# moddyz/stereo-to-multiview-cuda

Measured on AMD Instinct MI355X. Metric: stereo->8-view frames/sec @1080p d=64; cost-agg HBM GB/s vs roofline, higher is better.
Workload: dtype f32; 1 GPU; 1920x1080 synthetic stereo frame, D=64, zd=32, full stereo->8-view frame: cost init + cross aggregation + WTA + DCC/IRV x5/bilateral + 6 DIBR views + interlacing, one frame per GPU per step; stages=3, usd=34, lsd=17, views=8, aggregation=matrix pipe (stm_kernels_aggm.hip)

## Files before the change

include/stm_hip.h:

```cpp
#ifndef STM_HIP_H
#define STM_HIP_H

#ifdef __cplusplus
extern "C" {
#endif
#if defined(STM_BUILD) && defined(__GNUC__)
#pragma GCC visibility push(default)
#endif

int         stm_version(void);
void        stm_set_stream(void *hip_stream);
void       *stm_get_stream(void);
void        stm_set_error_mode(int mode);
const char *stm_last_error(void);
void        stm_release_workspace(void);
void        stm_prof_enable(int on);
void        stm_prof_reset(void);
int         stm_prof_read(const char *kernel, float *total_ms);
void        stm_set_agg_variant(int v);
int         stm_agg_path(int num_disp, int zero_disp, int num_rows, int num_cols, int usd, int stages);
void        stm_set_irv_paper_ratio(int on);
int         stm_set_irv_chunk(int entries);
int         stm_irv_path(int num_rows, int num_cols, int usd, int iterations, int device_flavour, int with_dcc);
int         stm_set_lens(int mode, double pitch, double slope, double centre);
int         stm_set_depth(int mode, float gain, float conv);
int         stm_set_depth_auto(float disp_lo, float disp_hi, float max_gain, int clip_permille, float rate, float *d_state);
int         stm_set_layout(int layout, int tiles_x, int tiles_y, int order, int filter);
void        stm_get_layout(int *out);
int         stm_set_output(int format, int matrix, int pitch, int uv_row);
void        stm_get_output(int out[4]);
void        stm_set_quilt_lds_limit(int bytes);
int         stm_set_packing(int packing, int swap, int filter, int gap);
void        stm_get_packing(int *out);
void        stm_set_ref_quirks(int on);

void stm_ci_adcensus(unsigned char *img_l, unsigned char *img_r, float **cost_l, float **cost_r,
                     float ad_coeff, float census_coeff, int num_disp, int zero_disp,
                     int num_rows, int num_cols, int elem_sz);
void stm_d_ci_adcensus(unsigned char *d_img_l, unsigned char *d_img_r,
                       float **d_adcensus_cost_l, float **d_adcensus_cost_r,
                       float **h_adcensus_cost_l, float **h_adcensus_cost_r,
                       float *d_adcensus_cost_memory,
                       float ad_coeff, float census_coeff, int num_disp, int zero_disp,
                       int num_rows, int num_cols, int elem_sz);

void stm_ca_cross(unsigned char *img, unsigned char **cross, float **cost, float **acost,
                  float ucd, float lcd, int usd, int lsd,
                  int num_disp, int num_rows, int num_cols, int elem_sz);
void stm_d_ca_cross(unsigned char *d_img, float **d_cost,
                    float **d_acost, float **h_acost, float *d_acost_memory,
                    unsigned char **d_cross,
                    float ucd, float lcd, int usd, int lsd,
                    int num_disp, int num_rows, int num_cols, int elem_sz);
// ... 227 lines not shown
```

stereo-to-multiview-cuda_amd/_lib.py:

```python
import ctypes as C
import os

HERE = os.path.dirname(os.path.abspath(__file__))
LIB_PATH = os.path.join(HERE, "libstm_hip.so")
if os.environ.get("STM_LIB") == "timing":
    LIB_PATH = os.path.join(HERE, "libstm_hip_timing.so")

u8p = C.POINTER(C.c_uint8)
f32p = C.POINTER(C.c_float)
u32p = C.POINTER(C.c_uint32)
u8pp = C.POINTER(u8p)
f32pp = C.POINTER(f32p)
vp = C.c_void_p
i, f, d = C.c_int, C.c_float, C.c_double

PROTOS = {
    "stm_version": ([], i),
    "stm_set_stream": ([vp], None),
    "stm_get_stream": ([], vp),
    "stm_set_error_mode": ([i], None),
    "stm_last_error": ([], C.c_char_p),
    "stm_release_workspace": ([], None),
    "stm_prof_enable": ([i], None),
    "stm_prof_reset": ([], None),
    "stm_prof_read": ([C.c_char_p, f32p], i),
    "stm_set_agg_variant": ([i], None),
    "stm_agg_path": ([i, i, i, i, i, i], i),
    "stm_set_irv_paper_ratio": ([i], None),
    "stm_set_irv_chunk": ([i], i),
    "stm_irv_path": ([i, i, i, i, i, i], i),
    "stm_set_ref_quirks": ([i], None),
    "stm_set_lens": ([i, d, d, d], i),
    "stm_set_layout": ([i, i, i, i, i], i),
    "stm_get_layout": ([C.POINTER(C.c_int)], None),
    "stm_set_output": ([i, i, i, i], i),
    "stm_get_output": ([C.POINTER(C.c_int)], None),
    "stm_set_quilt_lds_limit": ([i], None),
    "stm_set_packing": ([i, i, i, i], i),
    "stm_get_packing": ([C.POINTER(C.c_int)], None),
    "stm_set_depth": ([i, f, f], i),
    "stm_set_depth_auto": ([f, f, f, i, f, vp], i),
    "stm_ci_adcensus": ([u8p, u8p, f32pp, f32pp, f, f, i, i, i, i, i], None),
    "stm_d_ci_adcensus": ([vp, vp, vp, vp, f32pp, f32pp, vp, f, f, i, i, i, i, i], None),
    "stm_ca_cross": ([u8p, u8pp, f32pp, f32pp, f, f, i, i, i, i, i, i], None),
    "stm_d_ca_cross": ([vp, vp, vp, f32pp, vp, vp, f, f, i, i, i, i, i, i], None),
    "stm_dc_wta": ([f32pp, f32p, i, i, i, i], None),
    "stm_d_dc_wta": ([vp, vp, i, i, i, i], None),
    "stm_dc_subpixel": ([f32pp, f32p, i, i, i, i], None),
    "stm_d_dc_subpixel": ([vp, vp, i, i, i, i], None),
    "stm_dc_hslo": ([f32pp, f32p, u8p, u8p, f, f, f, i, i, i, i, i], None),
    "stm_d_dc_hslo": ([vp, vp, vp, vp, f, f, f, i, i, i, i, i], None),
    "stm_dr_dcc": ([u8p, u8p, f32p, f32p, i, i], None),
    "stm_d_dr_dcc": ([vp, vp, vp, vp, i, i], None),
    "stm_dr_irv": ([f32p, u8p, u8pp, i, f, i, i, i, i, i, i], None),
    "stm_d_dr_irv": ([vp, vp, vp, i, f, i, i, i, i, i, i], None),
    "stm_dr_interp": ([f32p, u8p, u8p, i, i, i], None),
    "stm_d_dr_interp": ([vp, vp, vp, i, i, i], None),
    "stm_filter_bilateral_1": ([f32p, i, f, f, i, i, i], None),
    "stm_d_filter_bilateral_1": ([vp, i, f, f, i, i, i], None),
    "stm_filter_gaussian_1": ([f32p, i, f, i, i], None),
# ... 95 lines not shown
```

stereo-to-multiview-cuda_amd/csrc/stm_api.hip:

```cpp
#include "stm_common.h"
#include <initializer_list>
#include <mutex>
#include "../../include/stm_hip.h"

#include <map>
#include <stdio.h>
#include <stdlib.h>
#include <string.h>
#include <tuple>
#include <vector>

using namespace stm;

namespace {

struct DevTable {
    float *d = nullptr;
    size_t n = 0;
};
std::map<std::tuple<int, int, float, float>, DevTable> g_tables;

int cur_dev()
{
    int dev = 0;
// ... 96 lines not shown
        }
    return true;
}


void core_ci(const u8 *d_img_l, const u8 *d_img_r, Vol cl, Vol cr, uint32_t *pk_l, uint32_t *pk_r, float ad_coeff,
             float census_coeff, int D, int zd, int H, int W, int elem_sz, bool packed_ready = false,
             uint32_t **census_out = nullptr, uint32_t *const *census_ready = nullptr)
{
    size_t HW = (size_t)H * W;
    uint32_t *cen_l = census_ready ? census_ready[0] : Workspace::get<uint32_t>(HW), *cen_r = census_ready ? census_ready[1] : Workspace::get<uint32_t>(HW);
    if (!packed_ready) {
        launch_pack_bgrx(d_img_l, pk_l, H, W, elem_sz);
        launch_pack_bgrx(d_img_r, pk_r, H, W, elem_sz);
    }
    if (!census_ready) launch_census32_pair(pk_l, cen_l, pk_r, cen_r, H, W);
    if (census_out) {
        census_out[0] = cen_l;
        census_out[1] = cen_r;
        return;
    }
    const float *lut = rho_table(ad_coeff, census_coeff);
    launch_cost_init(pk_l, pk_r, cen_l, cen_r, cl, cr, lut, lut + 768, D, zd, H, W);
    if (ref_quirks()) launch_cost_quirks(pk_l, pk_r, cen_l, cen_r, cl, cr, lut, lut + 768, D, zd, H, W);
}

static bool agg_on_matrix_pipe(int usd, int H, int W) { return (agg_variant() / 10000) % 10 != 1 && aggm_supports(usd, H, W); }
static bool stages_hslo(int stages) { return (stages & 0x100) != 0; }
static bool stages_subpix(int stages) { return (stages & 0x200) != 0; }
int frame_agg_path(int D, int zd, int H, int W, int usd, int stages)
{
    if (D < 1 || H < 1 || W < 1 || !agg_on_matrix_pipe(usd, H, W)) return 0;
    return 1 | aggm_frame_path(D, zd, H, W, usd, stages_hslo(stages), stages_subpix(stages));
}
void core_agg(Vol cost, Vol scratch, const Arms &a, int D, int H, int W, int usd)
{
    if (agg_on_matrix_pipe(usd, H, W) && launch_aggm_stage(cost, cost, a.up, a.down, a.left, a.right, D, H, W, usd)) return;
    if (!scratch.base && !scratch.tab) scratch = vol_slab(Workspace::get<float>((size_t)D * H * W), (size_t)H * W);
    launch_agg_h(cost, scratch, a.left, a.right, D, H, W);
    launch_agg_v(scratch, cost, a.up, a.down, D, H, W, usd);
    launch_agg_v(cost, scratch, a.up, a.down, D, H, W, usd);
    launch_agg_h(scratch, cost, a.left, a.right, D, H, W);
}
Arms carve_arms(size_t HW)
{
    u8 *m = Workspace::get<u8>(4 * HW);
    return Arms{m, m + HW, m + 2 * HW, m + 3 * HW};
}
Arms arms_from_table(unsigned char **d_cross)
{
    u8 *h[4];
    STM_CHECK(hipMemcpyAsync(h, d_cross, sizeof h, hipMemcpyDeviceToHost, stream()));
    sync();
    return Arms{h[0], h[1], h[2], h[3]};
}

void core_bilateral(float *d_img, int radius, float sigma_color, float sigma_spatial, int H, int W, int D)
{
    size_t HW = (size_t)H * W;
    float *tmp = Workspace::get<float>(HW);
    launch_bilateral(d_img, tmp, gauss2d_table(radius, sigma_spatial), gauss1d_table(D, sigma_color), radius, H, W, D);
    STM_CHECK(hipMemcpyAsync(d_img, tmp, HW * sizeof(float), hipMemcpyDeviceToDevice, stream()));
}

void core_dbm(u8 *d_out, const u8 *d_l, const u8 *d_r, const float *disp_l, const float *disp_r, const float *mask_l,
              const float *mask_r, float shift, int H, int W, int elem_sz, int g_radius, float g_sigma, bool linear = false)
// ... 1345 lines not shown
}

bool frame_dims_ok(const char *fn, int num_rows, int num_cols_sbs, int num_cols, int num_rows_out, int num_cols_out, int elem_sz,
                   int num_views, int num_disp)
{
    return args_ok(fn, {{"num_rows", num_rows, 1}, {"num_cols_sbs", num_cols_sbs, 1}, {"num_cols", num_cols, 1},
                        {"num_rows_out", num_rows_out, 1}, {"num_cols_out", num_cols_out, 1}, {"elem_sz", elem_sz, 3},
                        {"num_views", num_views, 2}, {"num_disp", num_disp, 1}});
}

bool frame_packing_ok(const char *fn, int num_rows, int num_cols_sbs, int num_cols)
{
    const Packing pk = packing();
    return !pk.on() || packing_args_ok(fn, pk, num_rows, num_cols_sbs, num_cols, "num_cols", false, 0, 0, 0);
}
bool packing_unsupported(const char *fn)
{
    if (!packing().on()) return false;
    char msg[200];
    snprintf(msg, sizeof msg, "%s: a packing is set on this thread (stm_set_packing), which this call does not support: use d_adcensus_stm, "
             "d_adcensus_stm_t or d_adcensus_stm_nv12", fn);
    fail(msg, "packing", __FILE__, __LINE__);
    return true;
}

}

extern "C" {

int stm_agg_path(int num_disp, int zero_disp, int num_rows, int num_cols, int usd, int stages)
{
    return frame_agg_path(num_disp, zero_disp, num_rows, num_cols, usd, stages);
}

void stm_d_adcensus_stm(unsigned char *d_img_sbs, float *d_disp_l, float *d_disp_r, unsigned char *d_interlaced,
                        int num_rows, int num_cols_sbs, int num_cols, int num_rows_out, int num_cols_out, int elem_sz,
                        int num_views, float angle, int num_disp, int zero_disp, float ad_coeff, float census_coeff,
                        float ucd, float lcd, int usd, int lsd, int thresh_s, float thresh_h, int stages)
{
    if (!frame_dims_ok("d_adcensus_stm", num_rows, num_cols_sbs, num_cols, num_rows_out, num_cols_out, elem_sz, num_views, num_disp)) return;
    if (!frame_packing_ok("d_adcensus_stm", num_rows, num_cols_sbs, num_cols)) return;
    if (stages & 0x2000) {
        fail("d_adcensus_stm: stages 0x2000 (temporal stabilisation) needs the history arguments of d_adcensus_stm_t", "stages", __FILE__,
             __LINE__);
        return;
    }
    frame_device("d_adcensus_stm", d_img_sbs, d_disp_l, d_disp_r, d_interlaced, num_rows, num_cols_sbs, num_cols, num_rows_out, num_cols_out,
                 elem_sz, num_views, angle, num_disp, zero_disp, ad_coeff, census_coeff, ucd, lcd, usd, lsd, thresh_s, thresh_h, stages, nullptr);
}

void stm_d_adcensus_stm_t(unsigned char *d_img_sbs, float *d_disp_l, float *d_disp_r, unsigned char *d_interlaced,
                          int num_rows, int num_cols_sbs, int num_cols, int num_rows_out, int num_cols_out, int elem_sz,
                          int num_views, float angle, int num_disp, int zero_disp, float ad_coeff, float census_coeff,
                          float ucd, float lcd, int usd, int lsd, int thresh_s, float thresh_h, int stages,
                          unsigned char *d_prev_img_sbs, float *d_prev_disp_l, float *d_prev_disp_r, float alpha, int thresh_color,
                          float thresh_disp)
{
    const char *fn = "d_adcensus_stm_t";
    if (!frame_dims_ok(fn, num_rows, num_cols_sbs, num_cols, num_rows_out, num_cols_out, elem_sz, num_views, num_disp)) return;
    if (!frame_packing_ok(fn, num_rows, num_cols_sbs, num_cols)) return;
    TemporalHist hist = {d_prev_img_sbs, d_prev_disp_l, d_prev_disp_r, alpha, thresh_color, thresh_disp};
    bool run = false;
    if (stages & 0x2000) {
        const int nset = (d_prev_img_sbs != nullptr) + (d_prev_disp_l != nullptr) + (d_prev_disp_r != nullptr);
        const size_t HW = (size_t)num_rows * num_cols;
        if (!temporal_params_ok(fn, alpha, thresh_color, thresh_disp)) return;
// ... 503 lines not shown
```

stereo-to-multiview-cuda_amd/csrc/stm_common.h:

```cpp
#pragma once
#include <hip/hip_runtime.h>
#include <stddef.h>
#include <stdint.h>

typedef unsigned char u8;

namespace stm {

void fail(const char *what, const char *expr, const char *file, int line);
bool failed();
void clear_failed();
struct ApiNest { ApiNest(); ~ApiNest(); };
bool api_outermost();
void release_host_frame_bufs();
bool nv12_args_ok(const char *fn, int num_rows, int num_cols_sbs, int num_cols, const char *cols_name, int pitch_y, int pitch_uv, int matrix);
#define STM_CHECK(expr)                                                                  \
    do {                                                                                 \
        hipError_t _e = (expr);                                                          \
        if (_e != hipSuccess) ::stm::fail(hipGetErrorString(_e), #expr, __FILE__, __LINE__); \
    } while (0)
#define STM_CHECK_LAUNCH() STM_CHECK(hipGetLastError())
#define STM_LAUNCH(...)                                     \
    do {                                                    \
        if (!::stm::failed()) hipLaunchKernelGGL(__VA_ARGS__); \
// ... 222 lines not shown
                      const float *blend, u8 *out, int N, float y_interval, float inv_y_interval, int ymod, int Hin, int Win, int Hout,
                      int Wout, int elem_sz, int variant, bool linear = false);
void launch_mux(const u8 *const *d_views, u8 *out, int N, float y_interval, float inv_y_interval, int ymod,
                int Hin, int Win, int Hout, int Wout, int elem_sz, int variant);
void launch_mux_lens(const u8 *const *d_views, u8 *out, int N, const Lens &ln, int Hin, int Win, int Hout, int Wout, int elem_sz);
void launch_synth_mux_lens(const u8 *img_l, const u8 *img_r, const float *disp_l, const float *disp_r, const float *mask_l,
                           const float *mask_r, const float *blend, u8 *out, int N, const Lens &ln, int Hin, int Win, int Hout, int Wout,
                           int elem_sz, bool linear);
void launch_synth_mux_depth(const u8 *img_l, const u8 *img_r, const float *disp_l, const float *disp_r, const float *mask_l,
                            const float *mask_r, const float *blend, u8 *out, int N, const Lens &ln, float inv_y_interval, int ymod,
                            float gain, float conv, const float *state, int Hin, int Win, int Hout, int Wout, int elem_sz, bool linear);
void launch_quilt(const u8 *const *d_views, u8 *out, int N, const Layout &lo, int Hin, int Win, int Hout, int Wout, int elem_sz);
void launch_synth_quilt(const u8 *img_l, const u8 *img_r, const float *disp_l, const float *disp_r, const float *mask_l, const float *mask_r,
                        const float *blend, u8 *out, int N, const Layout &lo, int depth_mode, float gain, float conv, const float *state,
                        int Hin, int Win, int Hout, int Wout, int elem_sz, bool linear, const Nv12Out *nv = nullptr);
void launch_depth_fit(float *state, uint32_t *hist, const float *disp_l, const float *disp_r, int H, int W, float disp_lo, float disp_hi,
                      float max_gain, int clip_permille, float rate, bool fresh);
struct PQViews {
    const uint32_t *pk[2], *cen[2];
    float *a[2], *b[2];
    const u8 *armU[2], *armD[2], *armL[2], *armR[2];
    float *disp[2];
};
size_t pq_volume_floats(int D, int H, int W);
bool aggm_supports(int usd, int H, int W);
void launch_aggm_frame(const uint32_t *const *pk, const uint32_t *const *cen, const float *lut, float *const *vol_a, float *const *vol_b,
                       const u8 *const *armU, const u8 *const *armD, const u8 *const *armL, const u8 *const *armR, float *const *disp,
                       int D, int zd, int H, int W, int usd, bool keep_volume = false, uint32_t *htab_ready = nullptr, uint32_t *vtab_ready = nullptr,
                       bool v2_read_later = false);
size_t aggm_frame_htab_dwords(int D, int H, int W, int usd, bool keep_volume);
size_t aggm_frame_vtab_dwords(int D, int zd, int H, int W, int usd, bool keep_volume, bool v2_read_later, int *rec, int *top, bool *col);
bool aggm_frame_px(int D, int zd, int H, int W, int usd, bool keep_volume, bool v2_read_later);
int aggm_frame_path(int D, int zd, int H, int W, int usd, bool keep_volume, bool v2_read_later);
bool launch_aggm_stage(Vol in, Vol out, const u8 *armU, const u8 *armD, const u8 *armL, const u8 *armR, int D, int H, int W, int usd);
size_t aggm_stage_bytes(int D, int H, int W, int usd);
bool aggh_supports(int usd, int D);
size_t aggh_table_dwords(int nviews, int H, int W);
void launch_hwin_table(PQViews &v, int nviews, uint32_t *tab, int H, int W);
void launch_pq_hsr(PQViews &v, int nviews, const uint32_t *tab, int D, int zd, int H, int W, bool px = false);
bool aggv_supports(int usd);
int aggv_table_top();
int aggv_table_rec();
void launch_pq_v12q(PQViews &v, int nviews, const uint32_t *tab, int rec, int H, int W, int G, int NC);
void launch_pq_v12r(PQViews &v, int nviews, const uint32_t *tab, int H, int W, int G);
void launch_vcol_table(PQViews &v, int nviews, uint32_t *tab, int H, int W);
size_t aggv_col_table_dwords(int nviews, int H, int W);
void launch_to_pq(Vol in, float *pq, int D, int H, int W, uint32_t *odd = nullptr);
void launch_from_pq(const float *pq, Vol out, int D, int H, int W);
void launch_hslo_wta(int nviews, const Vol *cost, const u8 *const *img_a, const u8 *const *img_b, const int *osign,
                     float *const *disp, float T, float H1, float H2, int D, int zd, int H, int W, int elem_sz);
void launch_hslo_wta_pq(int nviews, float *const *cost_pq, float *const *acc_pq, const u8 *const *img_a, const u8 *const *img_b,
                        const int *osign, float *const *disp, float T, float H1, float H2, int D, int zd, int H, int W, int elem_sz);

void rho_luts(float ad_coeff, float census_coeff, float *lut_ad , float *lut_census );
void gaussian_kernel_2d(float *kernel, int radius, float sigma);
void gaussian_kernel_1d(float *kernel, int size, float sigma);
float mux_y_interval(int num_views, float angle, int elem_sz);

}
```

stereo-to-multiview-cuda_amd/csrc/stm_kernels_aggm.hip:

```cpp
#include "stm_hwin.h"

namespace stm {

typedef float f4 __attribute__((ext_vector_type(4)));

#define STM_MFMA16(m, b, acc, abid) __builtin_amdgcn_mfma_f32_16x16x1f32(m, b, acc, 2, abid, 0)
typedef float f16v __attribute__((ext_vector_type(16)));
typedef uint32_t u4v __attribute__((ext_vector_type(4)));
#define STM_MASKF(m) (__builtin_amdgcn_inverse_ballot_w64(m) ? 1.0f : 0.0f)
#define STM_BLOAD(rsrc, voff) __builtin_bit_cast(f4, __builtin_amdgcn_raw_buffer_load_b128(rsrc, voff, 0, 2))


template <int N> __device__ __forceinline__ float row_ror_f(float v)
{
    return __builtin_bit_cast(float, __builtin_amdgcn_update_dpp(0, __builtin_bit_cast(int, v), 0x120 + N, 0xf, 0xf, false));
}
template <int N> __device__ __forceinline__ int row_ror_i(int v) { return __builtin_amdgcn_update_dpp(0, v, 0x120 + N, 0xf, 0xf, false); }
__device__ __forceinline__ int wave_min_i(int v)
{
    v = min(v, row_ror_i<8>(v)); v = min(v, row_ror_i<4>(v)); v = min(v, row_ror_i<2>(v)); v = min(v, row_ror_i<1>(v));
    return min(min(__builtin_amdgcn_readlane(v, 0), __builtin_amdgcn_readlane(v, 16)),
               min(__builtin_amdgcn_readlane(v, 32), __builtin_amdgcn_readlane(v, 48)));
}
__device__ __forceinline__ int wave_max_i(int v)
// ... 636 lines not shown
#pragma unroll
                for (int cl = 0; cl < 4; ++cl) {
                    const f4 o = {acc[4 * cl], acc[4 * cl + 1], acc[4 * cl + 2], acc[4 * cl + 3]};
                    if (!STM_DBG(dbg, 4)) STM_BSTORE(rout[cl], (X0 >> 2) * 256 + l * 16, o);
                }
            } else {
#pragma unroll
                for (int k = 0; k < 16; ++k)
                    if (!STM_DBG(dbg, 4))
                        __builtin_amdgcn_raw_buffer_store_b32(__builtin_bit_cast(uint32_t, (float)acc[k]), rpx,
                                                              (X0 + 4 * lb + (k & 3)) * 256 + (16 * (k >> 2) + dd) * 4, 0, 2);
            }
        }
        if (more) STM_HC_COSTS((sq + 1) & 1, 4 * NW * (sq + 1) + NG - 4 * NW)
        __syncthreads();
        if (more) {
            int sl = slot0 + w;
            if (sl >= NJ) sl -= NJ;
#pragma unroll
            for (int k = 0; k < 4; ++k) tile[(k * NJ + sl) * 64 + l] = cst[k];
            STM_HC_STAGE(sq & 1)
            STM_HC_SN(sq + 1)
            slot0 += NW;
            if (slot0 >= NJ) slot0 -= NJ;
        }
        __syncthreads();
    }
  }
#undef STM_HC_FETCH
#undef STM_HC_STAGE
#undef STM_HC_COSTS
#undef STM_HC_ARMS
#undef STM_HC_SN
}

constexpr int VT_EV = 2 * 255 + 32;
__global__ __launch_bounds__(256) void stm_k_vwin_table(PQViews v, uint32_t *__restrict__ tab, int rec, int H, int W, int G, int nT, int top)
{
    __shared__ unsigned long long ev_all[4][VT_EV];
    const int l = threadIdx.x & 63, wv = threadIdx.x >> 6, g = blockIdx.x * 4 + wv, u = blockIdx.y, view = blockIdx.z;
    if (g >= G) return;
    unsigned long long *ev = ev_all[wv];
    const u8 *__restrict__ armU = view ? v.armU[1] : v.armU[0], *__restrict__ armD = view ? v.armD[1] : v.armD[0];
    const int b = l >> 4, i = l & 15, y = u * 16 + i, x = 4 * g + b;
    int s0 = 0, nn = 0;
    if (y < H && x < W) {
        const int aU = armU[(size_t)y * W + x], aD = armD[(size_t)y * W + x];
        s0 = y - aU;
        nn = aU + aD;
    }
    vwin_build(tab + ((size_t)(view * nT + u) * G + g) * rec, ev, u, top, s0, nn);
}

typedef __attribute__((address_space(4))) const uint32_t ctab32;
typedef __attribute__((address_space(4))) const unsigned long long ctab64;
struct V12Quad { f4 c; unsigned long long m0, m1, m2, m3; };
struct V12Sweep {
    const f4 *p;
    ctab64 *mk;
    int qs, n_it;
    V12Quad A;
};
#define STM_V12_LOAD(S, Q, RQ)                                                      \
    {                                                                               \
        Q.c = *S.p;                                                                 \
        Q.m0 = S.mk[0]; Q.m1 = S.mk[1]; Q.m2 = S.mk[2]; Q.m3 = S.mk[3];             \
// ... 229 lines not shown
static int hc_waves(int D, int zd, int usd)
{
    constexpr int NW = 8, NWC = 12;
    const int NC = (D + 15) / 16;
    const int HG = ((usd + 3) / 4 + 2) & ~1, NG = 4 * NW + 2 * HG, NGc = 4 * NWC + 2 * HG;
    int pad = zd > D - 1 - zd ? zd : D - 1 - zd;
    pad = (pad < 0 ? 0 : pad) + 15;
    const size_t smem_hc = (size_t)4 * NGc * 256 + 16 * NWC * 4 + 8 * NWC + (size_t)(2 * 16 * NWC + 2 * (16 * NWC + 2 * pad)) * 8 + (768 + 72) * 4;
    const size_t smem_hc8 = (size_t)4 * NG * 256 + 16 * NW * 4 + 8 * NW + (size_t)(2 * 16 * NW + 2 * (16 * NW + 2 * pad)) * 8 + (768 + 72) * 4;
    const bool hc_ok = (agg_variant() / 1000000) % 10 != 1 && (agg_variant() / 1000) % 10 == 0 && (NC <= 4 || (agg_variant() / 10) % 10 != 2);
    if (hc_ok && smem_hc <= 80 * 1024 && 16 * NWC + 2 * pad <= 64 * NWC) return NWC;
    if (hc_ok && smem_hc8 <= 80 * 1024 && 16 * NW + 2 * pad <= 64 * NW) return NW;
    return 0;
}

static int row_split(int nseg) { return nseg > 24 ? cdiv(nseg, 16) : 1; }
static bool chain_vregs(int usd) { return aggv_supports(usd) && (agg_variant() / 10000000) % 10 != 1; }
static bool chain_hregs(bool wta, int usd, int D) { return wta && aggh_supports(usd, D) && (agg_variant() / 100000000) % 10 != 1; }

static bool chain_px(bool from_costs, bool wta, int D, int zd, int usd)
{
    if (usd > 255) usd = 255;
    const int NC = (D + 15) / 16;
    return from_costs && NC == 4 && chain_vregs(usd) && (agg_variant() / 10000000) % 10 == 0 && chain_hregs(wta, usd, D) &&
           hc_waves(D, zd, usd) != 0;
}
bool aggm_frame_px(int D, int zd, int H, int W, int usd, bool keep_volume, bool v2_read_later)
{
    (void)H;
    (void)W;
    return !v2_read_later && chain_px(true, !keep_volume, D, zd, usd);
}

struct ChainPlan {
    bool regs, hregs;
    int hcw;
    int hc_nseg, hc_spl;
};
static ChainPlan chain_plan(bool from_costs, bool wta, int D, int zd, int W, int usd)
{
    ChainPlan c;
    c.regs = chain_vregs(usd);
    c.hregs = chain_hregs(wta, usd, D);
    const bool fuse_cost = from_costs && (agg_variant() / 1000000) % 10 != 1;
    c.hcw = fuse_cost ? hc_waves(D, zd, usd) : 0;
    c.hc_nseg = c.hcw ? cdiv(W, 16 * c.hcw) : 0;
    c.hc_spl = row_split(c.hc_nseg);
    return c;
}
int aggm_frame_path(int D, int zd, int H, int W, int usd, bool keep_volume, bool v2_read_later)
{
    if (usd > 255) usd = 255;
    const ChainPlan c = chain_plan(true, !keep_volume, D, zd, W, usd);
    return (aggm_frame_px(D, zd, H, W, usd, keep_volume, v2_read_later) ? 2 : 0) | (c.regs ? 4 : 0) | (c.hregs ? 8 : 0) | (c.hcw << 8) |
           (c.hc_spl > 1 ? 1 << 16 : 0);
}

static void aggm_chain(PQViews &v, int nviews, bool from_costs, bool wta, const float *lut, int D, int zd, int H, int W, int usd,
                       uint32_t *htab_ready = nullptr, uint32_t *vtab_ready = nullptr, bool px = false)
{
    const int G = (W + 3) / 4, NC = (D + 15) / 16;
    if (usd > 255) usd = 255;
    constexpr int NW = 8;
    const int HG = ((usd + 3) / 4 + 2) & ~1, NG = 4 * NW + 2 * HG;
    const int nseg = cdiv(W, 16 * NW), nblk = ((nseg * H * nviews + 7) / 8) * 8;
    const size_t smem_h = (size_t)4 * NG * 256 + 16 * NW * 4;
    const int dbgh = timing_knobs();
    int pad = zd > D - 1 - zd ? zd : D - 1 - zd;
    pad = (pad < 0 ? 0 : pad) + 15;
    const size_t smem_cost = smem_h + (size_t)(4 * NG * 4 + 4 * pad + 768 + 72) * 4;
    const bool fuse_cost = from_costs && (agg_variant() / 1000000) % 10 != 1;
    const int spl = row_split(nseg);
    const ChainPlan plan = chain_plan(from_costs, wta, D, zd, W, usd);
    const bool streaming = NG / 4 >= NW && (agg_variant() / 10) % 10 != 1 && (NC <= 4 || (agg_variant() / 10) % 10 != 2);
    constexpr int NTP = 3, TS = 16 * NTP;
    const int UQ = (usd + 3) & ~3, nT = (H + 15) / 16;
    const bool regs = plan.regs;
    const int rec = regs ? aggv_table_rec() : 8 + 8 * ((2 * usd + 21) / 4 + 2);
    const int LAG = (UQ + TS - 1) / TS + 1;
    const int RQ1 = (TS + 2 * UQ) / 4, RQ2 = (TS * (LAG + 1) + UQ) / 4;
    uint32_t *vtab = regs && vtab_ready ? vtab_ready : Workspace::get<uint32_t>(px ? aggv_col_table_dwords(nviews, H, W) : (size_t)nviews * nT * G * rec);
    const bool hregs = plan.hregs;
    uint32_t *htab = !hregs ? nullptr : htab_ready ? htab_ready : Workspace::get<uint32_t>(aggh_table_dwords(nviews, H, W));
    {
        if (!(regs && vtab_ready)) {
            ProfScope p("pq_vtab");
            if (px) launch_vcol_table(v, nviews, vtab, H, W);
            else STM_LAUNCH(stm_k_vwin_table, dim3(cdiv(G, 4), nT, nviews), dim3(256), 0, stream(), v, vtab, rec, H, W, G, nT, regs ? aggv_table_top() : -1);
            STM_CHECK_LAUNCH();
        }
        if (hregs && !htab_ready) {
            ProfScope p("pq_htab");
            launch_hwin_table(v, nviews, htab, H, W);
        }
    }
    if (from_costs && !fuse_cost) {
        ProfScope p("pq_cost");
        const size_t smem = (size_t)(2 * PC_TX + 2 * (PC_TX + 2 * pad) + 768 + 72) * 4;
        allow_lds_m((const void *)stm_k_pq_cost, smem);
        STM_LAUNCH(stm_k_pq_cost, dim3(cdiv(W, PC_TX), H, nviews), dim3(PC_TX), smem, stream(), v, lut, D, zd, H, W, G, NC, pad);
        STM_CHECK_LAUNCH();
    }
    {
        ProfScope p("pq_h");
        constexpr int NWC = 12;
        const int NGc = 4 * NWC + 2 * HG;
        const size_t smem_c12 = (size_t)4 * NGc * 256 + 16 * NWC * 4 + (size_t)(4 * NGc * 4 + 4 * pad + 768 + 72) * 4;
        const size_t smem_hc = (size_t)4 * NGc * 256 + 16 * NWC * 4 + 8 * NWC + (size_t)(2 * 16 * NWC + 2 * (16 * NWC + 2 * pad)) * 8 + (768 + 72) * 4;
        const int nsegc = cdiv(W, 16 * NWC);
        const size_t smem_hc8 = (size_t)4 * NG * 256 + 16 * NW * 4 + 8 * NW + (size_t)(2 * 16 * NW + 2 * (16 * NW + 2 * pad)) * 8 + (768 + 72) * 4;
        const int hcw = plan.hcw;
#define STM_HC_LAUNCH(NWX, PXS, GRID, SMEM, NSEG, SPL)                                                                                      \
    {                                                                                                                                     \
        allow_lds_m((const void *)stm_k_pq_hc<NWX, PXS>, SMEM);                                                                            \
        STM_LAUNCH((stm_k_pq_hc<NWX, PXS>), GRID, dim3(64 * NWX), SMEM, stream(), v, D, zd, H, W, G, NC, HG, NSEG, SPL, lut, pad, dbgh);    \
    }
        if (hcw == NWC) {
            const dim3 grid(nviews * H * plan.hc_spl);
            if (px) STM_HC_LAUNCH(NWC, true, grid, smem_hc, plan.hc_nseg, plan.hc_spl)
            else STM_HC_LAUNCH(NWC, false, grid, smem_hc, plan.hc_nseg, plan.hc_spl)
        } else if (hcw == NW) {
            const dim3 grid(nviews * H * plan.hc_spl);
            if (px) STM_HC_LAUNCH(NW, true, grid, smem_hc8, plan.hc_nseg, plan.hc_spl)
            else STM_HC_LAUNCH(NW, false, grid, smem_hc8, plan.hc_nseg, plan.hc_spl)
        } else if (fuse_cost && smem_c12 <= 80 * 1024 && (agg_variant() / 1000) % 10 != 1) {
            const int nblkc = ((nsegc * H * nviews + 7) / 8) * 8;
            allow_lds_m((const void *)stm_k_pq_h<NWC, false, true>, smem_c12);
            STM_LAUNCH((stm_k_pq_h<NWC, false, true>), dim3(nblkc), dim3(64 * NWC), smem_c12, stream(), v, D, zd, H, W, G, NC, HG, nsegc, dbgh, lut, pad, nviews);
        } else if (fuse_cost) {
            allow_lds_m((const void *)stm_k_pq_h<NW, false, true>, smem_cost);
            STM_LAUNCH((stm_k_pq_h<NW, false, true>), dim3(nblk), dim3(64 * NW), smem_cost, stream(), v, D, zd, H, W, G, NC, HG, nseg, dbgh, lut, pad, nviews);
        } else if (streaming) {
            allow_lds_m((const void *)stm_k_pq_hs<NW, false>, smem_h);
            STM_LAUNCH((stm_k_pq_hs<NW, false>), dim3(nviews * H * spl), dim3(64 * NW), smem_h, stream(), v, D, zd, H, W, G, NC, HG, nseg, spl, dbgh);
        } else {
            allow_lds_m((const void *)stm_k_pq_h<NW, false, false>, smem_h);
            STM_LAUNCH((stm_k_pq_h<NW, false, false>), dim3(nblk), dim3(64 * NW), smem_h, stream(), v, D, zd, H, W, G, NC, HG, nseg, dbgh, lut, 0, nviews);
        }
#undef STM_HC_LAUNCH
        STM_CHECK_LAUNCH();
    }
    {
        ProfScope p("pq_v12");
        if (px) {
            launch_pq_v12r(v, nviews, vtab, H, W, G);
        } else if (regs) {
            launch_pq_v12q(v, nviews, vtab, rec, H, W, G, NC);
        } else {
            const size_t smem = (size_t)(RQ1 + RQ2) * 1024;
            allow_lds_m((const void *)stm_k_pq_v12t<NTP>, smem);
// ... 90 lines not shown
```

stereo-to-multiview-cuda_amd/device_api.py:

```python
import ctypes as C

import torch

from ._lib import f32p, f32pp, lib


def _use_current_stream():
    lib().stm_set_stream(C.c_void_p(torch.cuda.current_stream().cuda_stream))


def _p(t):
    return C.c_void_p(t.data_ptr())


STAGE_SUBPIXEL = 0x200
STAGE_INTERP = 0x400
STAGE_LINEAR_WARP = 0x800
STAGE_GUIDED_UP = 0x1000
STAGE_TEMPORAL = 0x2000
TEMPORAL_DEFAULTS = (0.5, 24, 1.5)


class FrameParams:

    def __init__(self, num_disp=64, zero_disp=32, num_views=8, angle=18.43, ad_coeff=10.0, census_coeff=30.0,
                 ucd=6.0, lcd=20.0, usd=34, lsd=17, thresh_s=20, thresh_h=0.4, out_rows=None, out_cols=None):
        self.num_disp, self.zero_disp, self.num_views, self.angle = num_disp, zero_disp, num_views, angle
        self.ad_coeff, self.census_coeff = ad_coeff, census_coeff
        self.ucd, self.lcd, self.usd, self.lsd = ucd, lcd, usd, lsd
        self.thresh_s, self.thresh_h = thresh_s, thresh_h
        self.out_rows, self.out_cols = out_rows, out_cols


AGG_MATRIX_PIPE, AGG_PX, AGG_VREGS, AGG_HREGS, AGG_SPLIT = 1, 2, 4, 8, 1 << 16


def agg_path(num_disp, zero_disp, num_rows, num_cols, usd, stages=3):
    return int(lib().stm_agg_path(int(num_disp), int(zero_disp), int(num_rows), int(num_cols), int(usd), int(stages)))


def agg_path_waves(path):
    return (int(path) >> 8) & 0xff


IRV_PRUNE, IRV_RUNS, IRV_CHAIN = 1, 2, 4


def irv_path(num_rows, num_cols, usd, iterations=5, device_flavour=True, with_dcc=False):
    return int(lib().stm_irv_path(int(num_rows), int(num_cols), int(usd), int(iterations), int(bool(device_flavour)), int(bool(with_dcc))))


def irv_path_tile_sh(path):
    return (int(path) >> 8) & 0xf


def irv_path_chunk(path):
    return (int(path) >> 16) & 0x1f


def set_irv_chunk(entries=0):
    if int(lib().stm_set_irv_chunk(int(entries))) != 0:
        raise ValueError("stm_set_irv_chunk(%d) refused: %s" % (entries, lib().stm_last_error().decode()))


def set_lens(mode, pitch=0.0, slope=0.0, centre=0.0):
    if int(lib().stm_set_lens(int(mode), float(pitch), float(slope), float(centre))) != 0:
        raise ValueError("stm_set_lens(%d, %g, %g, %g) refused: %s" % (mode, pitch, slope, centre, lib().stm_last_error().decode()))


def set_layout(layout=0, tiles_x=1, tiles_y=1, order=0, filter=0):
    if int(lib().stm_set_layout(int(layout), int(tiles_x), int(tiles_y), int(order), int(filter))) != 0:
        raise ValueError("stm_set_layout(%d, %d, %d, %d, %d) refused: %s"
                         % (layout, tiles_x, tiles_y, order, filter, lib().stm_last_error().decode()))


# ... 411 lines not shown
```

Baseline: 658.1 frames/s.

## Add fused two-view cost+horizontal aggregation kernel with sliding cost ring

Adds a new first-pass kernel that computes AD-census costs for both views in one 12-wave block. It keeps a sliding LDS ring of costs across 96-pixel segments and performs the horizontal cross aggregation with MFMA, double-buffering pixel fetches and arm loads for the next segment. The aim is to reuse overlapping cost columns across segments and serve both views from one launch instead of separate per-view horizontal-cost kernels. The trade-off is a large LDS footprint, a more complex synchronisation schedule, and new path selection logic plus a query API.

```diff
diff --git a/include/stm_hip.h b/include/stm_hip.h
--- a/include/stm_hip.h
+++ b/include/stm_hip.h
@@ -19,6 +19,7 @@
 int         stm_prof_read(const char *kernel, float *total_ms);
 void        stm_set_agg_variant(int v);
 int         stm_agg_path(int num_disp, int zero_disp, int num_rows, int num_cols, int usd, int stages);
+int         stm_first_pass_path(int num_disp, int zero_disp, int num_rows, int num_cols, int usd, int stages);
 void        stm_set_irv_paper_ratio(int on);
 int         stm_set_irv_chunk(int entries);
 int         stm_irv_path(int num_rows, int num_cols, int usd, int iterations, int device_flavour, int with_dcc);
diff --git a/stereo-to-multiview-cuda_amd/_lib.py b/stereo-to-multiview-cuda_amd/_lib.py
--- a/stereo-to-multiview-cuda_amd/_lib.py
+++ b/stereo-to-multiview-cuda_amd/_lib.py
@@ -26,6 +26,7 @@
     "stm_prof_read": ([C.c_char_p, f32p], i),
     "stm_set_agg_variant": ([i], None),
     "stm_agg_path": ([i, i, i, i, i, i], i),
+    "stm_first_pass_path": ([i, i, i, i, i, i], i),
     "stm_set_irv_paper_ratio": ([i], None),
     "stm_set_irv_chunk": ([i], i),
     "stm_irv_path": ([i, i, i, i, i, i], i),
diff --git a/stereo-to-multiview-cuda_amd/csrc/stm_api.hip b/stereo-to-multiview-cuda_amd/csrc/stm_api.hip
--- a/stereo-to-multiview-cuda_amd/csrc/stm_api.hip
+++ b/stereo-to-multiview-cuda_amd/csrc/stm_api.hip
@@ -152,6 +152,11 @@
 {
     if (D < 1 || H < 1 || W < 1 || !agg_on_matrix_pipe(usd, H, W)) return 0;
     return 1 | aggm_frame_path(D, zd, H, W, usd, stages_hslo(stages), stages_subpix(stages));
+}
+int frame_first_pass_path(int D, int zd, int H, int W, int usd, int stages)
+{
+    if (D < 1 || H < 1 || W < 1 || !agg_on_matrix_pipe(usd, H, W)) return 0;
+    return aggm_frame_hc2_parts(D, zd, H, W, usd, stages_hslo(stages), stages_subpix(stages));
 }
 void core_agg(Vol cost, Vol scratch, const Arms &a, int D, int H, int W, int usd)
 {
@@ -1563,6 +1568,10 @@
 {
     return frame_agg_path(num_disp, zero_disp, num_rows, num_cols, usd, stages);
 }
+int stm_first_pass_path(int num_disp, int zero_disp, int num_rows, int num_cols, int usd, int stages)
+{
+    return frame_first_pass_path(num_disp, zero_disp, num_rows, num_cols, usd, stages);
+}
 
 void stm_d_adcensus_stm(unsigned char *d_img_sbs, float *d_disp_l, float *d_disp_r, unsigned char *d_interlaced,
                         int num_rows, int num_cols_sbs, int num_cols, int num_rows_out, int num_cols_out, int elem_sz,
diff --git a/stereo-to-multiview-cuda_amd/csrc/stm_common.h b/stereo-to-multiview-cuda_amd/csrc/stm_common.h
--- a/stereo-to-multiview-cuda_amd/csrc/stm_common.h
+++ b/stereo-to-multiview-cuda_amd/csrc/stm_common.h
@@ -278,6 +278,7 @@
 size_t aggm_frame_vtab_dwords(int D, int zd, int H, int W, int usd, bool keep_volume, bool v2_read_later, int *rec, int *top, bool *col);
 bool aggm_frame_px(int D, int zd, int H, int W, int usd, bool keep_volume, bool v2_read_later);
 int aggm_frame_path(int D, int zd, int H, int W, int usd, bool keep_volume, bool v2_read_later);
+int aggm_frame_hc2_parts(int D, int zd, int H, int W, int usd, bool keep_volume, bool v2_read_later);
 bool launch_aggm_stage(Vol in, Vol out, const u8 *armU, const u8 *armD, const u8 *armL, const u8 *armR, int D, int H, int W, int usd);
 size_t aggm_stage_bytes(int D, int H, int W, int usd);
 bool aggh_supports(int usd, int D);
diff --git a/stereo-to-multiview-cuda_amd/csrc/stm_kernels_aggm.hip b/stereo-to-multiview-cuda_amd/csrc/stm_kernels_aggm.hip
--- a/stereo-to-multiview-cuda_amd/csrc/stm_kernels_aggm.hip
+++ b/stereo-to-multiview-cuda_amd/csrc/stm_kernels_aggm.hip
@@ -692,6 +692,188 @@
 #undef STM_HC_COSTS
 #undef STM_HC_ARMS
 #undef STM_HC_SN
+}
+
+constexpr int HC2_TX = 96, HC2_SR = HC2_TX + 64, HC2_HALO = 40, HC2_RING = 256, HC2_FRONT = HC2_TX + HC2_HALO;
+typedef const float __attribute__((address_space(3))) *hc2_lds_cf;
+constexpr size_t HC2_SMEM =(size_t)(HC2_RING + 3) * 256 + 2 * HC2_TX * 4 + 12 * 8 + (size_t)(2 * HC2_TX + 2 * HC2_SR) * 8 + (768 + 72) * 4;
+__global__ __launch_bounds__(768, 6) void stm_k_pq_hc2(PQViews v, int D, int zd, int H, int W, int G, int nseg, int spl,
+                                                       const float *__restrict__ lut_g, int dbg)
+{
+    constexpr int NW = 12, NT = 64 * NW, TX = HC2_TX, SR = HC2_SR;
+    extern __shared__ f4 lds4[];
+    float *ring = (float *)lds4;
+    uint32_t *sn = (uint32_t *)(ring + (HC2_RING + 3) * 64);
+    int2 *sg = (int2 *)(sn + 2 * TX);
+    uint2 *s_l = (uint2 *)(sg + NW), *s_r = s_l + 2 * TX;
+    float *s_lut_ad = (float *)(s_r + 2 * SR), *s_lut_c = s_lut_ad + 768;
+    const int tid = threadIdx.x, l = tid & 63, w = __builtin_amdgcn_readfirstlane(tid >> 6);
+    const int lb = l >> 4, dd = l & 15;
+    const int part = blockIdx.x % spl, y = blockIdx.x / spl;
+    const int seg_per = (nseg + spl - 1) / spl, seg0 = part * seg_per, seg1 = min(nseg, seg0 + seg_per);
+    if (seg0 >= seg1) return;
+    const int view = w >= NW / 2, wt = view ? w - NW / 2 : w;
+    f4 *__restrict__ out = (f4 *)(view ? v.b[1] : v.b[0]);
+    const uint32_t *__restrict__ pk_l = v.pk[0], *__restrict__ pk_r = v.pk[1], *__restrict__ cen_l = v.cen[0], *__restrict__ cen_r = v.cen[1];
+    const int aview = tid >= TX, apx = aview ? tid - TX : tid;
+    const u8 *__restrict__ armL = aview ? v.armL[1] : v.armL[0], *__restrict__ armR = aview ? v.armR[1] : v.armR[0];
+    const size_t row = (size_t)y * W;
+    const uint32_t rowbytes = (uint32_t)G * 256u;
+    for (int i = tid; i < 768 + 65; i += NT) s_lut_ad[i] = lut_g[i];
+    uint2 sl = make_uint2(0, 0), sr = make_uint2(0, 0);
+    int aLn = 0, aRn = 0;
+    float cst[8];
+    const __amdgpu_buffer_rsrc_t rpx = __builtin_amdgcn_make_buffer_rsrc((void *)(out + (size_t)y * G * 64), 0, 4u * rowbytes, 0x00020000);
+#define STM_HC2_FETCH(P0)                                                                          \
+    {                                                                                              \
+        if (tid < TX) {                                                                            \
+            const int gx = min(max((P0) + tid, 0), W - 1);                                         \
+            sl = make_uint2(pk_l[row + gx], cen_l[row + gx]);                                      \
+        }                                                                                          \
+        if (tid < SR) {                                                                            \
+            const int gx = min(max((P0) - zd + tid, 0), W - 1);                                    \
+            sr = make_uint2(pk_r[row + gx], cen_r[row + gx]);                                      \
+        }                                                                                          \
+    }
+#define STM_HC2_STAGE(B)                                           \
+    {                                                              \
+        if (tid < TX) s_l[(B) * TX + tid] = sl;                    \
+        if (tid < SR) s_r[(B) * SR + tid] = sr;                    \
+    }
+#define STM_HC2_COSTS(B)                                                                                                  \
+    {                                                                                                                     \
+        const uint2 *lp = s_l + (B) * TX + 8 * w, *rp = s_r + (B) * SR + 8 * w + l;                                       \
+        _Pragma("unroll") for (int k = 0; k < 8; ++k) {                                                                   \
+            const uint2 o = lp[k], q = rp[k];                                                                             \
+            const float a = s_lut_ad[__builtin_amdgcn_sad_u8(o.x, q.x, 0u)], c = s_lut_c[hamdist_q1(o.y, q.y)];           \
+            cst[k] = l < D ? a + c : 0.f;                                                                                 \
+        }                                                                                                                 \
+    }
+#define STM_HC2_WRITE(P0)                                                              \
+    _Pragma("unroll") for (int k = 0; k < 8; ++k) {                                    \
+        const int rp_ = ((P0) + 8 * w + k) & (HC2_RING - 1);              \
+        ring[rp_ * 64 + l] = cst[k];                                                   \
+        if (rp_ < 3) ring[(HC2_RING + rp_) * 64 + l] = cst[k];                         \
+    }
+#define STM_HC2_ARMS(S)                                                         \
+    if (tid < 2 * TX) {                                                         \
+        const int x = min((S) * TX + apx, W - 1);                               \
+        aLn = armL[row + x];                                                    \
+        aRn = armR[row + x];                                                    \
+    }
+#define STM_HC2_SN(S)                                                                                                      \
+    if (tid < 2 * TX) {                                                                                                    \
+        const int x = (S) * TX + apx, org = (S) * TX - HC2_HALO;                                                           \
+         \
+        const int srel_ = x < W ? x - aLn - org : x - org, nn_ = x < W ? aLn + aRn : 0;                                    \
+        sn[tid] = (uint32_t)srel_ | ((uint32_t)nn_ << 16);                                                                 \
+                           \
+        int lo_ = nn_ ? (srel_ >> 2) : 0x7fffffff, hi_ = nn_ ? ((srel_ + nn_ + 3) >> 2) : -0x7fffffff;                     \
+        lo_ = min(lo_, row_ror_i<8>(lo_)); lo_ = min(lo_, row_ror_i<4>(lo_)); lo_ = min(lo_, row_ror_i<2>(lo_)); lo_ = min(lo_, row_ror_i<1>(lo_)); \
+        hi_ = max(hi_, row_ror_i<8>(hi_)); hi_ = max(hi_, row_ror_i<4>(hi_)); hi_ = max(hi_, row_ror_i<2>(hi_)); hi_ = max(hi_, row_ror_i<1>(hi_)); \
+        if ((tid & 15) == 0) sg[tid >> 4] = make_int2(lo_, hi_ - lo_);                                                     \
+    }
+    const int front0 = TX * seg0 + HC2_FRONT + zd;
+    for (int r0 = 0; r0 < HC2_RING; r0 += TX) {
+        const int p0 = front0 - HC2_RING + r0;
+        STM_HC2_FETCH(p0)
+        __syncthreads();
+        STM_HC2_STAGE(0)
+        __syncthreads();
+        if (r0 + 8 * w < HC2_RING) {
+            STM_HC2_COSTS(0)
+            STM_HC2_WRITE(p0)
+        }
+    }
+    __syncthreads();
+    {
+        STM_HC2_FETCH(front0)
+        STM_HC2_STAGE((seg0 + 1) & 1)
+        STM_HC2_ARMS(seg0)
+        STM_HC2_SN(seg0)
+    }
+    __syncthreads();
+    const int shear = view ? min(l, D - 1) - zd : 0;
+    for (int sq = seg0; sq < seg1; ++sq) {
+        const int X0 = sq * TX + 16 * wt;
+        const int front = TX * sq + HC2_FRONT + zd;
+        const bool more = sq + 1 < seg1;
+        if (more) {
+            STM_HC2_FETCH(front + TX)
+            STM_HC2_ARMS(sq + 1)
+        }
+        if (X0 < W) {
+            const uint32_t e = sn[16 * w + dd];
+            const int srel = (int)(e & 0xffffu), nn = (int)(e >> 16);
+            const int2 sgw = sg[w];
+            const int G0r = __builtin_amdgcn_readfirstlane(sgw.x);
+            const int n_it = STM_DBG(dbg, 1) ? 0 : __builtin_amdgcn_readfirstlane(sgw.y);
+            f16v acc;
+            if (n_it > 0) {
+                uint32_t a = ((((unsigned)(sq * TX - HC2_HALO + 4 * G0r - shear) << 8) + 4u * l) & 0xffffu);
+                int t = 4 * G0r + lb - srel;
+#define STM_HS_NEXT(C)                                                        \
+    {                                                                         \
+        const hc2_lds_cf r_ = (hc2_lds_cf)(size_t)a;                          \
+        C.x = r_[0]; C.y = r_[64]; C.z = r_[128]; C.w = r_[192];              \
+        asm("v_add_u16_e32 %0, 0x400, %1" : "=v"(a) : "v"(a));                \
+    }
+#define STM_HS_MFMA(C)                                                          \
+    {                                                                           \
+        const float m = ((unsigned)t < (unsigned)nn) ? 1.0f : 0.0f;             \
+        t += 4;                                                                 \
+        acc = STM_MFMA16(m, C.x, acc, 0);                                       \
+        acc = STM_MFMA16(m, C.y, acc, 1);                                       \
+        acc = STM_MFMA16(m, C.z, acc, 2);                                       \
+        acc = STM_MFMA16(m, C.w, acc, 3);                                       \
+    }
+                f4 ca, cb;
+                STM_HS_NEXT(ca)
+                STM_HS_NEXT(cb)
+                {
+                    const float m = ((unsigned)t < (unsigned)nn) ? 1.0f : 0.0f;
+                    t += 4;
+                    const f16v z = {0.f, 0.f, 0.f, 0.f, 0.f, 0.f, 0.f, 0.f, 0.f, 0.f, 0.f, 0.f, 0.f, 0.f, 0.f, 0.f};
+                    acc = STM_MFMA16(m, ca.x, z, 0);
+                    acc = STM_MFMA16(m, ca.y, acc, 1);
+                    acc = STM_MFMA16(m, ca.z, acc, 2);
+                    acc = STM_MFMA16(m, ca.w, acc, 3);
+                }
+                int it = 1;
+                for (; it + 2 <= n_it; it += 2) {
+                    STM_HS_NEXT(ca)
+                    STM_HS_MFMA(cb)
+                    STM_HS_NEXT(cb)
+                    STM_HS_MFMA(ca)
+                }
+                if (it < n_it) STM_HS_MFMA(cb)
+#undef STM_HS_NEXT
+#undef STM_HS_MFMA
+            } else {
+#pragma unroll
+                for (int i = 0; i < 16; ++i) acc[i] = 0.f;
+            }
+#pragma unroll
+            for (int k = 0; k < 16; ++k)
+                if (!STM_DBG(dbg, 4))
+                    __builtin_amdgcn_raw_buffer_store_b32(__builtin_bit_cast(uint32_t, (float)acc[k]), rpx,
+                                                          (X0 + 4 * lb + (k & 3)) * 256 + (16 * (k >> 2) + dd) * 4, 0, 2);
+        }
+        if (more) STM_HC2_COSTS((sq + 1) & 1)
+        __syncthreads();
+        if (more) {
+            STM_HC2_WRITE(front)
+            STM_HC2_STAGE(sq & 1)
+            STM_HC2_SN(sq + 1)
+        }
+        __syncthreads();
+    }
+#undef STM_HC2_FETCH
+#undef STM_HC2_STAGE
+#undef STM_HC2_COSTS
+#undef STM_HC2_WRITE
+#undef STM_HC2_ARMS
+#undef STM_HC2_SN
 }
 
 constexpr int VT_EV = 2 * 255 + 32;
@@ -987,12 +1169,23 @@
     return !v2_read_later && chain_px(true, !keep_volume, D, zd, usd);
 }
 
+constexpr int HC2_SLOTS = 2 * 256;
+static int hc2_parts(bool px, int D, int zd, int H, int W, int usd)
+{
+    const int HG = ((usd + 3) / 4 + 2) & ~1;
+    if (!px || (agg_variant() / 1000000) % 10 == 2 || hc_waves(D, zd, usd) != 12) return 0;
+    if (zd < 0 || zd >= D || D > 64 || 4 * HG > HC2_HALO) return 0;
+    if (cdiv(W, HC2_TX) < 8 || H >= 8 * HC2_SLOTS) return 1;
+    return 2 * row_split(cdiv(W, 2 * HC2_TX));
+}
+
 struct ChainPlan {
     bool regs, hregs;
     int hcw;
     int hc_nseg, hc_spl;
+    int hc2_spl;
 };
-static ChainPlan chain_plan(bool from_costs, bool wta, int D, int zd, int W, int usd)
+static ChainPlan chain_plan(bool from_costs, bool wta, int D, int zd, int H, int W, int usd, bool px)
 {
     ChainPlan c;
     c.regs = chain_vregs(usd);
@@ -1001,14 +1194,21 @@
     c.hcw = fuse_cost ? hc_waves(D, zd, usd) : 0;
     c.hc_nseg = c.hcw ? cdiv(W, 16 * c.hcw) : 0;
     c.hc_spl = row_split(c.hc_nseg);
+    c.hc2_spl = fuse_cost && c.hcw ? hc2_parts(px, D, zd, H, W, usd) : 0;
     return c;
 }
 int aggm_frame_path(int D, int zd, int H, int W, int usd, bool keep_volume, bool v2_read_later)
 {
     if (usd > 255) usd = 255;
-    const ChainPlan c = chain_plan(true, !keep_volume, D, zd, W, usd);
+    const ChainPlan c = chain_plan(true, !keep_volume, D, zd, H, W, usd, false);
     return (aggm_frame_px(D, zd, H, W, usd, keep_volume, v2_read_later) ? 2 : 0) | (c.regs ? 4 : 0) | (c.hregs ? 8 : 0) | (c.hcw << 8) |
            (c.hc_spl > 1 ? 1 << 16 : 0);
+}
+
+int aggm_frame_hc2_parts(int D, int zd, int H, int W, int usd, bool keep_volume, bool v2_read_later)
+{
+    if (usd > 255) usd = 255;
+    return chain_plan(true, !keep_volume, D, zd, H, W, usd, aggm_frame_px(D, zd, H, W, usd, keep_volume, v2_read_later)).hc2_spl;
 }
 
 static void aggm_chain(PQViews &v, int nviews, bool from_costs, bool wta, const float *lut, int D, int zd, int H, int W, int usd,
@@ -1026,7 +1226,7 @@
     const size_t smem_cost = smem_h + (size_t)(4 * NG * 4 + 4 * pad + 768 + 72) * 4;
     const bool fuse_cost = from_costs && (agg_variant() / 1000000) % 10 != 1;
     const int spl = row_split(nseg);
-    const ChainPlan plan = chain_plan(from_costs, wta, D, zd, W, usd);
+    const ChainPlan plan = chain_plan(from_costs, wta, D, zd, H, W, usd, px && nviews == 2);
     const bool streaming = NG / 4 >= NW && (agg_variant() / 10) % 10 != 1 && (NC <= 4 || (agg_variant() / 10) % 10 != 2);
     constexpr int NTP = 3, TS = 16 * NTP;
     const int UQ = (usd + 3) & ~3, nT = (H + 15) / 16;
@@ -1070,7 +1270,10 @@
         allow_lds_m((const void *)stm_k_pq_hc<NWX, PXS>, SMEM);                                                                            \
         STM_LAUNCH((stm_k_pq_hc<NWX, PXS>), GRID, dim3(64 * NWX), SMEM, stream(), v, D, zd, H, W, G, NC, HG, NSEG, SPL, lut, pad, dbgh);    \
     }
-        if (hcw == NWC) {
+        if (plan.hc2_spl) {
+            allow_lds_m((const void *)stm_k_pq_hc2, HC2_SMEM);
+            STM_LAUNCH(stm_k_pq_hc2, dim3(H * plan.hc2_spl), dim3(768), HC2_SMEM, stream(), v, D, zd, H, W, G, cdiv(W, HC2_TX), plan.hc2_spl, lut, dbgh);
+        } else if (hcw == NWC) {
             const dim3 grid(nviews * H * plan.hc_spl);
             if (px) STM_HC_LAUNCH(NWC, true, grid, smem_hc, plan.hc_nseg, plan.hc_spl)
             else STM_HC_LAUNCH(NWC, false, grid, smem_hc, plan.hc_nseg, plan.hc_spl)
diff --git a/stereo-to-multiview-cuda_amd/device_api.py b/stereo-to-multiview-cuda_amd/device_api.py
--- a/stereo-to-multiview-cuda_amd/device_api.py
+++ b/stereo-to-multiview-cuda_amd/device_api.py
@@ -41,6 +41,10 @@
 
 def agg_path_waves(path):
     return (int(path) >> 8) & 0xff
+
+
+def first_pass_path(num_disp, zero_disp, num_rows, num_cols, usd, stages=3):
+    return int(lib().stm_first_pass_path(int(num_disp), int(zero_disp), int(num_rows), int(num_cols), int(usd), int(stages)))
 
 
 IRV_PRUNE, IRV_RUNS, IRV_CHAIN = 1, 2, 4
```

After: 671.4 frames/s, median of 6. +2.0%, better.
